# thu-nics/Rad-NeRF

Measured on AMD Instinct MI355X. Metric: million samples/s fwd+bwd, 8192 rays, model_zoo_size=2; rgb L∞ vs ref, higher is better.
Workload: dtype f16/f32

## Files before the change

include/radnerf.h:

```cpp
#ifndef RADNERF_H
#define RADNERF_H

#include <stdint.h>

#ifdef __cplusplus
extern "C" {
#endif

#define RN_ABI_VERSION 9
#define RN_FX_STATS_BYTES 640
int rn_version(void);
const char* rn_last_error(void);
const char* rn_abi_signatures(void);
void rn_set_debug_flags(int flags);
int rn_debug_cycles(unsigned long long* out);
int rn_set_level_pairing(uint64_t pairing);

int rn_ray_aabb_intersect(const float* rays_o, const float* rays_d, const float* centers,
                          const float* half_sizes, int64_t n_rays, int64_t n_voxels,
                          int32_t max_hits, int32_t* hit_cnt, float* hits_t,
                          int64_t* hits_voxel_idx, void* stream);

int rn_ray_sphere_intersect(const float* rays_o, const float* rays_d, const float* centers,
                            const float* radii, int64_t n_rays, int64_t n_spheres,
// ... 182 lines not shown
int rn_igrad_to_f32(int64_t n, int32_t* igrad_lo, int32_t* igrad_carry, const float* scale,
                    float* grid_grad, void* stream);

int rn_field_fwd_merged(const float* ts, const int32_t* ray_of, const float* rays_o,
                        const float* rays_d, const int32_t* seg_base, const int32_t* seg_count,
                        const int32_t* chunk_desc, int32_t* queue,
                        int64_t n_rays, int32_t n_models, const void* grid_f16,
                        const uint32_t* level_offset, const uint32_t* level_hsize,
                        const uint32_t* level_res, const float* level_scale,
                        const float* xyz_min, const float* extent, const void* frags,
                        float* sigma, float* rgb, void* feat_cache, const int32_t* mstart,
                        const int32_t* perm, int32_t blocks, int32_t threads, void* stream);

int rn_field_fwd_levels(const float* ts, const int32_t* ray_of, const float* rays_o,
                        const float* rays_d, const int32_t* seg_base, const int32_t* seg_count,
                        int64_t n_rays, int32_t n_models, const void* grid_f16,
                        const uint32_t* level_offset, const uint32_t* level_hsize,
                        const uint32_t* level_res, const float* level_scale,
                        const float* xyz_min, const float* extent, const void* frags,
                        float* sigma, float* rgb, void* feat_cache, const int32_t* mstart,
                        const int32_t* perm, uint32_t* planes, int64_t plane_stride, void* prep,
                        int32_t prep_ready, int32_t enc_blocks, int32_t mlp_blocks, int32_t* xq,
                        void* stream);

int rn_gate_fwd(const float* in0, const float* in1, int32_t stride, int64_t n_rays,
                int32_t n_models, const void* frags, float* gate, float* importance,
                int32_t n_blocks, void* stream);
int rn_gate_bwd(const float* in0, const float* in1, int32_t stride, int64_t n_rays,
                int32_t n_models, const void* frags, const float* dL_dgate, float* dw,
                int32_t n_params, const void* dinput_frags, float* dL_dinput,
                int32_t n_blocks, void* stream);

int rn_field_dinput(const float* xyzs, const float* dirs, int64_t n_samples, const float* ts,
                    const int32_t* ray_of, const float* rays_o, const float* rays_d,
                    const int32_t* seg_base, const int32_t* seg_count, int32_t n_models,
                    const void* grid_f16, const uint32_t* level_offset,
                    const uint32_t* level_hsize, const uint32_t* level_res,
                    const float* level_scale, const float* xyz_min, const float* extent,
                    const void* frags, const void* dinput_frags, const float* dL_dsigma,
                    const float* dL_drgb, const void* feat_cache, float* dL_dxyz,
                    float* dL_ddir, int32_t blocks_per_model, void* stream);
int rn_density_update_sampled(const void* grid_ptrs, const void* bitfield_ptrs, int32_t n_models,
                              int32_t cascades, int32_t grid_size, float scale,
                              float density_threshold, float decay, uint64_t seed,
                              const void* grid_f16, const uint32_t* level_offset,
                              const uint32_t* level_hsize, const uint32_t* level_res,
// ... 115 lines not shown
```

rad-nerf_amd/csrc/field.hip:

```cpp
#include "rn_field.h"
#include "rn_bin.h"
#include "rn_merge.h"
#include "rn_gradform.h"
#pragma clang fp contract(off)

static int g_field_dbg = 0;
__device__ unsigned long long g_rn_cyc[8];

namespace {

template <int MODE, int CACHE>
__global__ void __launch_bounds__(256, FWD_MIN_WAVES)
k_field_fwd(FieldArgs a) {
    __shared__ __attribute__((aligned(16))) rn_half sW[FIELD_FWD_FRAGS * RN_FRAG_HALFS];
    __shared__ LvTab sT;
    const int k = blockIdx.y;
    rn_block_copy16(sW, a.frags + (size_t)k * FIELD_FRAGS * RN_FRAG_HALFS,
                    FIELD_FWD_FRAGS * RN_FRAG_BYTES);
    lv_stage(sT, a.gm);
    __syncthreads();
    int64_t base, n;
    sample_range(a, MODE, k, base, n);
    const int64_t n_tiles = (n + 31) / 32;
    const int waves = blockDim.x / RN_WAVE;
// ... 1202 lines not shown
    return 0;
}

}
template <bool ABL, int DET>
static void launch_bwd_merged(int gm, int blocks, hipStream_t st, const FieldArgs& a,
                              const MergeArgs& m, const IntGrad& G, const FxGrad& F) {
#define MB_K(C, M) k_field_bwd_merged<C, ABL, M, DET><<<blocks, BWD_WAVES * 64, 0, st>>>(a, m, G, F)
    if constexpr (!DET) {
        if (gm == GM_BIN_F32) MB_K(CACHE_READ, GM_BIN_F32);
        if (gm == GM_BIN) MB_K(CACHE_READ, GM_BIN);
        if (gm == GM_FX) MB_K(CACHE_READ, GM_FX);
        if constexpr (!ABL) if (gm == GM_FX_REDO) MB_K(CACHE_READ, GM_FX_REDO);
    }
    if constexpr (!ABL) {
        if (gm == GM_INT) { if (a.feat) MB_K(CACHE_READ, GM_INT); else MB_K(CACHE_NONE, GM_INT); }
    }
    if constexpr (!DET) {
        if (gm == GM_F32) { if (a.feat) MB_K(CACHE_READ, GM_F32); else MB_K(CACHE_NONE, GM_F32); }
    }
#undef MB_K
}

static int field_bwd_merged(const char* who, bool det, const float* ts, const int32_t* ray_of,
                            const float* rays_o, const float* rays_d, const int32_t* seg_base,
                            const int32_t* seg_count, const int32_t* mstart, const int32_t* perm,
                            const int32_t* chunk_desc, int32_t* queue, int64_t n_rays,
                            int32_t n_models, int32_t max_samples, const void* grid_f16,
                            const uint32_t* level_offset, const uint32_t* level_hsize,
                            const uint32_t* level_res, const float* level_scale,
                            const float* xyz_min, const float* extent, const void* frags,
                            const float* dL_dsigma, const float* dL_drgb, float* grid_grad,
                            float* dw, const void* feat_cache, float* scratch,
                            int64_t scratch_rows, float* park, int32_t max_chunk, int32_t blocks,
                            int32_t* igrad_lo, int32_t* igrad_carry, const float* igrad_scale,
                            int32_t* fx_acc, const float* fx_scale, uint32_t* fx_stats,
                            const int32_t* fx_redo, int32_t fx_mode, void* gb_ctl,
                            uint32_t* gb_page_meta, uint64_t* gb_pages, int32_t gb_pool_pages,
                            void* stream) {
#define CHECK(cond, msg) RN_CHECK_ARG_AS(who, cond, msg)
    CHECK(!igrad_lo || (igrad_carry && igrad_scale), "integer mode needs carry and scale");
    CHECK(fx_mode >= GM_F32 && fx_mode <= GM_BIN_F32 && fx_mode != GM_INT, "fx_mode: 0, 2, 3, 4 or 5");
    const bool binned = gm_pages(fx_mode);
    CHECK(fx_mode != GM_FX || (fx_acc && fx_scale && fx_stats && feat_cache),
          "fixed-point mode needs acc, scale, stats and the encoding cache");
    CHECK(!binned || (fx_scale && fx_stats && feat_cache && gb_ctl && gb_page_meta && gb_pages &&
                      gb_pool_pages >= 1),
          "binned mode needs scale, stats, the encoding cache and the page pool");
    for (int l = 0; binned && l < RN_L; ++l)
        CHECK(level_hsize[l] <= (1u << GB_IDX_BITS) &&
              level_hsize[l] <= ((uint32_t)GB_MAX_BINS << GB_SLICE_BITS),
              "binned mode: a level has more than 2^20 entries");
    CHECK(fx_mode != GM_FX_REDO || (fx_redo && fx_scale && feat_cache),
          "fixed-point redo needs the redo flag, the step's scales and the encoding cache");
    CHECK(!(igrad_lo && fx_mode), "integer and fixed-point modes are exclusive");
    CHECK(n_rays >= 1 && n_models >= 1 && n_models <= MB_KMAX && blocks >= 1 &&
          max_samples >= 1 && max_chunk >= 1, "bad sizes");
    CHECK(scratch_rows >= (int64_t)max_chunk + (int64_t)n_models * max_samples,
          "scratch_rows must be >= max_chunk + n_models * max_samples");
    CHECK(ts && ray_of && rays_o && rays_d && seg_base && seg_count && mstart && perm &&
          chunk_desc && queue && grid_f16 && level_offset && level_hsize && level_res &&
          level_scale && xyz_min && extent && frags && dL_dsigma && dL_drgb && grid_grad && dw &&
          scratch && park, "null pointer");
    CHECK(fx_mode != GM_FX ||
          2ull * ((uint64_t)level_offset[RN_L - 1] + level_hsize[RN_L - 1]) <= (1ull << 28),
          "fixed-point mode: the grid has more than 2^28 gradient elements");
#undef CHECK
    FieldArgs a{};
    field_args_grid(a, grid_f16, level_offset, level_hsize, level_res, level_scale, xyz_min, extent,
                    frags);
    field_args_compact(a, ts, ray_of, rays_o, rays_d, seg_base, seg_count);
    a.dsigma = dL_dsigma; a.drgb = dL_drgb; a.grid_grad = grid_grad; a.dw = dw;
    a.feat = (rn_half*)feat_cache;
    MergeArgs m{};
    m.mstart = mstart; m.perm = perm; m.desc = chunk_desc; m.queue = queue; m.scratch = scratch;
    m.park = park; m.rows_cap = (int)scratch_rows; m.n_rays = (int)n_rays; m.n_models = n_models;
    hipStream_t st = (hipStream_t)stream;
    const size_t slots = (size_t)blocks * n_models * FIELD_PARAMS * sizeof(float);
    if (det) RN_CHECK_HIP_AS(who, hipMemsetAsync(dw, 0, slots, st), "dw_part reset");
    else RN_CHECK_HIP_AS(who, hipMemsetAsync(queue, 0, sizeof(int32_t), st), "ticket reset");
    IntGrad G{};
    if (igrad_lo) {
        G.bytes = 2 * a.grid_bytes;
        G.lo_ptr = igrad_lo; G.carry_ptr = igrad_carry; G.scale_ptr = igrad_scale;
    }
    if (binned) {
        RN_CHECK_HIP_AS(who, hipMemsetAsync(gb_ctl, 0, GB_CTL_RESET_BYTES, st), "page pool reset");
        G.ctl = (GbCtl*)gb_ctl; G.page_meta = gb_page_meta; G.pages = gb_pages;
        G.pool_pages = (uint32_t)gb_pool_pages;
    }
    FxGrad F{};
    F.acc = fx_acc; F.scale = fx_scale; F.redo = fx_redo;
    if (FxStats* S = reinterpret_cast<FxStats*>(fx_stats)) {
        F.vmax = S->vmax; F.qsum = S->qsum; F.wq = S->wq;
    }
    const int gm = fx_mode ? fx_mode : (igrad_lo ? GM_INT : GM_F32);
    const bool abl = RN_ABL && a.dbg && !det && gm != GM_INT && gm != GM_FX_REDO;
    if (abl) launch_bwd_merged<RN_ABL != 0, 0>(gm, blocks, st, a, m, G, F);
    else if (!det) launch_bwd_merged<false, 0>(gm, blocks, st, a, m, G, F);
    else launch_bwd_merged<false, 1>(gm, blocks, st, a, m, G, F);
    RN_CHECK_LAUNCH_AS(who);
    return 0;
}

extern "C" {
int rn_field_bwd_merged(const float* ts, const int32_t* ray_of, const float* rays_o,
                        const float* rays_d, const int32_t* seg_base, const int32_t* seg_count,
                        const int32_t* mstart, const int32_t* perm, const int32_t* chunk_desc,
                        int32_t* queue, int64_t n_rays, int32_t n_models, int32_t max_samples,
                        const void* grid_f16, const uint32_t* level_offset,
                        const uint32_t* level_hsize, const uint32_t* level_res,
                        const float* level_scale, const float* xyz_min, const float* extent,
                        const void* frags, const float* dL_dsigma, const float* dL_drgb,
                        float* grid_grad, float* dw, const void* feat_cache, float* scratch,
                        int64_t scratch_rows, float* park, int32_t max_chunk, int32_t blocks,
                        int32_t* igrad_lo, int32_t* igrad_carry, const float* igrad_scale,
                        int32_t* fx_acc, const float* fx_scale, uint32_t* fx_stats,
                        const int32_t* fx_redo, int32_t fx_mode, void* gb_ctl,
                        uint32_t* gb_page_meta, uint64_t* gb_pages, int32_t gb_pool_pages,
                        void* stream) {
    return field_bwd_merged(__func__, false, ts, ray_of, rays_o, rays_d, seg_base, seg_count,
// ... 10 lines not shown
                            const int32_t* seg_count, const int32_t* mstart, const int32_t* perm,
                            const int32_t* chunk_desc, const int32_t* queue, int64_t n_rays,
                            int32_t n_models, int32_t max_samples, const void* grid_f16,
                            const uint32_t* level_offset, const uint32_t* level_hsize,
                            const uint32_t* level_res, const float* level_scale,
                            const float* xyz_min, const float* extent, const void* frags,
                            const float* dL_dsigma, const float* dL_drgb, float* grid_grad,
                            float* dw_part, const void* feat_cache, float* scratch,
                            int64_t scratch_rows, float* park, int32_t max_chunk, int32_t blocks,
                            int32_t* igrad_lo, int32_t* igrad_carry, const float* igrad_scale,
                            void* stream) {
    RN_CHECK_ARG(igrad_lo && igrad_carry && igrad_scale,
                 "the deterministic backward needs igrad_lo, igrad_carry and igrad_scale");
    RN_CHECK_ARG(dw_part, "the deterministic backward needs dw_part");
    return field_bwd_merged(__func__, true, ts, ray_of, rays_o, rays_d, seg_base, seg_count,
                            mstart, perm, chunk_desc, const_cast<int32_t*>(queue), n_rays,
                            n_models, max_samples, grid_f16, level_offset, level_hsize, level_res,
                            level_scale, xyz_min, extent, frags, dL_dsigma, dL_drgb, grid_grad,
                            dw_part, feat_cache, scratch, scratch_rows, park, max_chunk, blocks,
                            igrad_lo, igrad_carry, igrad_scale, nullptr, nullptr, nullptr, nullptr,
                            GM_F32, nullptr, nullptr, nullptr, 0, stream);
}

}
```

rad-nerf_amd/csrc/field_fwd_merged.hip:

```cpp
#include "rn_field.h"
#include "rn_merge.h"
#pragma clang fp contract(off)

static uint64_t g_level_pairing = 0;

namespace {

#define FM_KMAX 8
#define FM_LDS_K 4
static_assert(FM_KMAX == MB_KMAX, "k_field_fwd_merged reads the plan's descriptors");

template <int CACHE, bool ENC_M, bool GW>
__global__ void __launch_bounds__(1024)
k_field_fwd_merged(FieldArgs a, MergeArgs m) {
    extern __shared__ __attribute__((aligned(16))) rn_half sWm[];
    __shared__ LvTab sT;
    __shared__ int32_t sCh[2][2 + 2 * FM_KMAX];
    const int K = m.n_models, B = m.n_rays;
    if (!GW) {
        for (int k = 0; k < K; ++k)
            rn_block_copy16(sWm + (size_t)k * FIELD_FWD_FRAGS * RN_FRAG_HALFS,
                            a.frags + (size_t)k * FIELD_FRAGS * RN_FRAG_HALFS,
                            FIELD_FWD_FRAGS * RN_FRAG_BYTES);
    }
// ... 182 lines not shown
            int k = kb;
            while (k < ke && u >= first[k + 1]) ++k;
            const int t = u - first[k];
            const int n_k = sSeg[1][k];
            const int i = t * 32 + c;
            const bool valid = i < n_k;
            const int64_t s = sSeg[0][k] + (valid ? i : 0);
            FwdState st;
            float ux, uy, uz;
            rn_lds_order();
            tile_forward_s<1, CACHE_PLANES>(a, sT, sWm + (size_t)(k - kb) * FIELD_FWD_FRAGS * RN_FRAG_HALFS,
                                            s, valid, a.feat ? cache_slot(a, s) : nullptr, st,
                                            ux, uy, uz);
            if (valid && h == 0) {
                a.sigma[s] = expf(st.g0);
                a.rgb[3 * s + 0] = sigmoidf(st.out[0]);
                a.rgb[3 * s + 1] = sigmoidf(st.out[1]);
                a.rgb[3 * s + 2] = sigmoidf(st.out[2]);
            }
        }
    }
}

}

extern "C" {

int rn_set_level_pairing(uint64_t pairing) {
    if (pairing != 0) {
        uint32_t seen = 0;
        for (int i = 0; i < 16; ++i) seen |= 1u << ((pairing >> (4 * i)) & 15u);
        RN_CHECK_ARG(seen == 0xffffu, "pairing: every level exactly once");
    }
    g_level_pairing = pairing;
    return 0;
}

int rn_field_fwd_merged(const float* ts, const int32_t* ray_of, const float* rays_o,
                        const float* rays_d, const int32_t* seg_base, const int32_t* seg_count,
                        const int32_t* chunk_desc, int32_t* queue,
                        int64_t n_rays, int32_t n_models, const void* grid_f16,
                        const uint32_t* level_offset, const uint32_t* level_hsize,
                        const uint32_t* level_res, const float* level_scale,
                        const float* xyz_min, const float* extent, const void* frags,
                        float* sigma, float* rgb, void* feat_cache, const int32_t* mstart,
                        const int32_t* perm, int32_t blocks, int32_t threads, void* stream) {
    RN_CHECK_ARG(n_rays >= 1 && n_models >= 1 && n_models <= FM_KMAX && blocks >= 1,
                 "bad sizes (n_models <= 8)");
    RN_CHECK_ARG(threads >= 64 && threads <= 1024 && threads % 64 == 0, "threads: 64..1024, waves");
// ... 76 lines not shown
```

rad-nerf_amd/csrc/rn_field.h:

```cpp
#pragma once
#include "rn_mlp.h"
#pragma clang fp contract(off)

#define RN_L 16
#define FIELD_FWD_FRAGS 24
#define FIELD_FRAGS 46
#define FIELD_PARAMS 9472
#define FIELD_DW_TILES 12
#ifndef FWD_MIN_WAVES
#define FWD_MIN_WAVES 2
#endif

struct GridMeta {
    uint32_t offset[RN_L];
    uint32_t hsize[RN_L];
    uint32_t res[RN_L];
    float scale[RN_L];
    uint32_t dense_mask;
    uint32_t pow2_mask;
};

struct FieldArgs {
    const float* xyzs; const float* dirs;
    const float* ts; const int32_t* ray_of; const float* rays_o; const float* rays_d;
// ... 401 lines not shown
template <int CACHE>
__device__ __forceinline__ void tile_forward_rays(const FieldArgs& a, const LvTab& T,
                                                  const rn_half* W, int64_t s, bool valid,
                                                  half8* fc, const float* sRays, int r0, int nr,
                                                  FwdState& st, float& ux, float& uy, float& uz) {
    float x = 0.f, y = 0.f, z = 0.f, dx = 1.f, dy = 0.f, dz = 0.f;
    if (valid) {
        const int r = a.ray_of[s];
        const float t = a.ts[s];
        const uint32_t q = (uint32_t)(r - r0);
        float ox, oy, oz;
        if (q < (uint32_t)nr) {
            typedef __attribute__((address_space(3))) const float lds_f;
            lds_f* p = (lds_f*)sRays + 6 * q;
            ox = p[0]; oy = p[1]; oz = p[2]; dx = p[3]; dy = p[4]; dz = p[5];
        } else {
            ox = a.rays_o[3 * r]; oy = a.rays_o[3 * r + 1]; oz = a.rays_o[3 * r + 2];
            dx = a.rays_d[3 * r]; dy = a.rays_d[3 * r + 1]; dz = a.rays_d[3 * r + 2];
        }
        x = fmaf(t, dx, ox);
        y = fmaf(t, dy, oy);
        z = fmaf(t, dz, oz);
    }
    tile_forward_pos<CACHE>(a, T, W, x, y, z, dx, dy, dz, valid, fc, st, ux, uy, uz);
}

template <int CACHE>
__device__ __forceinline__ void tile_forward_pos(const FieldArgs& a, const LvTab& T, const rn_half* W,
                                                 float x, float y, float z, float dx, float dy,
                                                 float dz, bool valid, half8* fc, FwdState& st,
                                                 float& ux, float& uy, float& uz) {
    const int h = rn_lane() >> 5;
    ux = unit_coord(x, a.xyz_min[0], a.extent[0]);
    uy = unit_coord(y, a.xyz_min[1], a.extent[1]);
    uz = unit_coord(z, a.xyz_min[2], a.extent[2]);
    if (CACHE == CACHE_PLANES) {
        if (valid && fc) { fc[0] = st.e0; fc[1] = st.e1; }
    } else if (CACHE == CACHE_READ || CACHE == CACHE_READ_NT) {
        st.e0 = rn_zero8(); st.e1 = rn_zero8();
        if (valid && CACHE == CACHE_READ) { st.e0 = fc[0]; st.e1 = fc[1]; }
        if (valid && CACHE == CACHE_READ_NT) {
            st.e0 = __builtin_nontemporal_load(fc);
            st.e1 = __builtin_nontemporal_load(fc + 1);
        }
    } else {
        if (rn_dbg(a.dbg) & 256) { st.e0 = rn_zero8(); st.e1 = rn_zero8(); asm volatile("" :: "v"(ux), "v"(uy), "v"(uz)); }
// ... 64 lines not shown
```

rad-nerf_amd/radnerf_amd/_lib.py:

```python
import ctypes
import os

_HERE = os.path.dirname(os.path.abspath(__file__))
LIB_PATH = os.environ.get("RADNERF_LIB", os.path.join(_HERE, "librn.so"))
ABLATION_LIB_PATH = os.environ.get("RADNERF_ABL_LIB", os.path.join(_HERE, "librn_abl.so"))

P = ctypes.c_void_p
I32 = ctypes.c_int32
I64 = ctypes.c_int64
F32 = ctypes.c_float
F64 = ctypes.c_double
U64 = ctypes.c_uint64

SIGNATURES = {
    "rn_ray_aabb_intersect": [P, P, P, P, I64, I64, I32, P, P, P, P],
    "rn_ray_sphere_intersect": [P, P, P, P, I64, I64, I32, P, P, P, P],
    "rn_raymarching_train_bw": [P, P, P, P, I64, P, P, P],
    "rn_ml_march_bw": [P, P, I64, I32, P, P, P, P, P, P],
    "rn_field_dinput": [P, P, I64, P, P, P, P, P, P, I32, P, P, P, P, P, P, P, P, P, P, P, P, P,
                        P, I32, P],
    "rn_field_density": [P, I64, P, P, P, P, P, P, P, P, P, P, P],
    "rn_debug_cycles": [P],
    "rn_set_level_pairing": [ctypes.c_uint64],
    "rn_density_update_sampled": [P, P, I32, I32, I32, F32, F32, F32, U64, P, P, P, P, P, P, P,
# ... 28 lines not shown
    "rn_bwd_plan": [P, P, P, P, P, I64, I32, I32, I32, I32, I32, I32, I32, P, P, P, P, P,
                    P, P, P, P, P, P],
    "rn_field_bwd_merged": [P, P, P, P, P, P, P, P, P, P, I64, I32, I32, P, P, P, P, P, P,
                            P, P, P, P, P, P, P, P, I64, P, I32, I32, P, P, P, P, P, P,
                            P, I32, P, P, P, I32, P],
    "rn_grid_fx_fold": [P, P, P, P, P, P, P, P, P, P],
    "rn_grid_bin_layout": [P],
    "rn_debug_gb_cycles": [P],
    "rn_grid_slice_bits": [P, P],
    "rn_grid_record_encode": [P, I64, P],
    "rn_grid_record_decode": [P, I64, P],
    "rn_grid_bin": [P, P, P, P, P, P, P, I32, I32, P],
    "rn_grid_sum": [P, P, P, P, P, P, I32, P, P, P, I32, I32, P],
    "rn_grid_bin_check": [P, P, P, P, P, P, P, I32, P, P, P, P, P],
    "rn_grid_binned_fold": [P, P, P, P, P, P, P, P, I32, P, P, P, P, P, P],
    "rn_render_test": [P, P, P, I64, I32, P, I64, I32, F32, F32, I32, I32, P, P, P, P, P, P, P,
                       P, F32, P, P, P, P, I32, P],
    "rn_seed_scale": [P, P, I32, P, P, P, P, P, P],
    "rn_igrad_to_f32": [I64, P, P, P, P, P],
    "rn_field_fwd_merged": [P, P, P, P, P, P, P, P, I64, I32, P, P, P, P, P, P, P, P, P, P, P,
                            P, P, I32, I32, P],
    "rn_field_fwd_levels": [P, P, P, P, P, P, I64, I32, P, P, P, P, P, P, P, P, P, P, P, P, P,
                            P, I64, P, I32, I32, I32, P, P],
    "rn_gate_fwd": [P, P, I32, I64, I32, P, P, P, I32, P],
    "rn_gate_bwd": [P, P, I32, I64, I32, P, P, P, I32, P, P, I32, P],
    "rn_nerf_loss": [P, P, P, P, P, P, I64, I32, F32, F32, F32, P, P, P, P, P, P],
    "rn_adam": [P, P, P, P, I64, F64, F64, F64, F64, I32, F32, P, I64, P],
    "rn_reduce_partials": [P, I32, I64, P, P],
    "rn_colsum_ordered": [P, I64, I32, P, P],
    "rn_field_bwd_merged_det": [P, P, P, P, P, P, P, P, P, P, I64, I32, I32, P, P, P, P, P, P,
                                P, P, P, P, P, P, P, P, I64, P, I32, I32, P, P, P, P],
    "rn_gate_bwd_det": [P, P, I32, I64, I32, P, P, P, I32, P, P, I32, P],
    "rn_nerf_loss_det": [P, P, P, P, P, P, I64, I32, F32, F32, F32, P, P, P, P, P, P, P],
    "rn_get_rays": [P, P, P, P, I64, P, P, P, P, P],
    "rn_get_rays_pose": [P, P, P, P, P, P, I64, P, P, P, P, P],
    "rn_get_rays_pose_bw": [P, P, P, P, P, I64, I64, P, P, P, P, P, P, P],
    "rn_sample_batch": [P, I32, I64, I64, P, P, P, P, P, U64, I64, I32, I64, I32, P, P, P, P, P,
                        P, P, P, P],
    "rn_ml_combine_test": [P, P, P, P, P, I64, I32, I64, P, P, P, P, P],
    "rn_image_sse": [P, P, I64, P, P, P],
    "rn_ssim": [P, P, I32, I32, I32, P, P, P, P],
    "rn_minmax_finite": [P, I64, I64, P, P, P],
    "rn_quantize_u8": [P, I64, P, P],
    "rn_colormap_u8": [P, I64, I64, P, P, I32, P, P],
    "rn_gate_map_u8": [P, I64, I32, P, I32, P, P],
    "rn_pack_f16": [P, I64, P, I64, I32, I64, P, P],
# ... 115 lines not shown
```

rad-nerf_amd/radnerf_amd/fused.py:

```python
import collections

import torch

from . import layout as LY
from ._lib import lib
from .networks import field_ptrs, model_bitfields

MAX_SAMPLES = 1024
NEAR_DISTANCE = 0.01
SEG_ALIGN = 128
FX_STATS_BYTES = 640
GM_F32, GM_FX, GM_FX_REDO, GM_BIN, GM_BIN_F32 = 0, 2, 3, 4, 5
NO_IG, NO_FX, NO_GB = (None, None, None), (None, None, None, None, GM_F32), (None, None, None, 0)


GB_SUM_FAULT = 18
GB_CTL_READ = GB_SUM_FAULT + 1


def clamp_split(split_level):
    return max(0, min(15, int(split_level)))


def _stream(dev):
# ... 10 lines not shown
        self.B, self.K, self.device = B, K, device
        cap = capacity or (B * K * max_samples + SEG_ALIGN * K)
        self.capacity = cap
        f = dict(device=device, dtype=torch.float32)
        i = dict(device=device, dtype=torch.int32)
        self.counts = torch.empty(K, B, **i)
        self.offsets = torch.empty(K, B, **i)
        self.seg = torch.zeros(2 * K + 2, **i)
        self.used = torch.empty(K, B, **i)
        self.ts = torch.empty(cap, **f)
        self.deltas = torch.empty(cap, **f)
        self.ray_of = torch.empty(cap, **i)
        self.sigma = torch.empty(cap, **f)
        self.rgb = torch.empty(cap, 3, **f)
        self.ws = torch.empty(cap, **f)
        self.dsigma = torch.empty(cap, **f)
        self.drgb = torch.empty(cap, 3, **f)
        self.opacity_k = torch.empty(K, B, **f)
        self.depth_k = torch.empty(K, B, **f)
        self.rgb_k = torch.empty(K, B, 3, **f)
        self.dgate = torch.empty(B, K, **f)
        self.stage_ts = torch.empty(K * B * max_samples, **f)
        self.stage_dt = torch.empty(K * B * max_samples, **f)
        self.feat = torch.empty((cap + 31) // 32 * 32, 32, device=device, dtype=torch.float16)
        self.mstart = torch.empty(B + 1, **i)
        self.perm = torch.empty(cap, **i)
        self.queue = torch.zeros(3, **i)
        self._bwd_scratch = None
        self._chunks = self._chunk_desc = None
        self._dist_k = None
        self._igrad = self._fx = self._bin = self._bin_ring = None
        self.fx_i = self._bin_n = 0
        self.dw_part = self.gate_part = None
        self.gate_dx = self.dxyz = self.ddir = self.drays_o = self.drays_d = None
        self.generation = 0

    @property
    def dist_k(self):
        if self._dist_k is None:
            self._dist_k = torch.empty(self.K, self.B, device=self.device, dtype=torch.float32)
        return self._dist_k

    def chunk_list(self, max_chunk, min_chunk, head_chunks=0, balance_blocks=0):
        cap = (head_chunks + self.capacity // max_chunk + self.capacity // (8 * min_chunk) +
               max_chunk // min_chunk + 3 + balance_blocks)
        if self._chunks is None or self._chunks.numel() < cap + 1:
            self._chunks = torch.empty(cap + 1, device=self.device, dtype=torch.int32)
            self._chunk_desc = torch.empty(cap + 1, 20, device=self.device, dtype=torch.int32)
        return cap, self._chunks

    def level_buffers(self, stream=None):
        rows = self.feat.shape[0]
        key = (str(self.device), int(stream) if stream is not None else 0)
        cur = _LEVEL_SCRATCH.get(key)
        if cur is None or cur[0].shape[1] < rows:
            cur = (torch.empty(16, rows, device=self.device, dtype=torch.int32),
                   torch.empty(rows, 4, device=self.device, dtype=torch.float32))
            _LEVEL_SCRATCH[key] = cur
        return cur

    def fx_buffers(self, n, device):
        if self._fx is None or self._fx[0].numel() != n:
            z = dict(device=device, dtype=torch.int32)
            self._fx = (torch.zeros(n, **z), torch.zeros(2, 16, device=device),
                        torch.zeros(FX_STATS_BYTES // 4, **z), torch.zeros(1, **z))
            self.fx_i = 0
        return self._fx

    def bin_pool(self, pages):
        b = self._bin
        if b is None or b["pages"] < pages:
            lay = lib().bin_layout()
            i = dict(device=self.device, dtype=torch.int32)
            self._bin = b = dict(
                pages=pages, page=lay["page"],
                ctl=torch.zeros(lay["ctl_bytes"] // 4, **i),
                meta=torch.zeros(pages, **i),
                recs=torch.empty(pages * lay["page"], device=self.device, dtype=torch.int64),
                desc=torch.empty(pages * lay["bins"], **i),
                lpages=torch.empty(16 * pages, **i))
        return b

# ... 17 lines not shown
    @property
    def meta(self):
        return self.seg[2 * self.K:]

    def n_samples(self):
        return int(self.meta[1].item())


class FusedMLRenderer:

    def __init__(self, model, gating_net, n_rays, device=None, fwd_blocks=None, bwd_blocks=None,
                 capacity=None, deterministic=False):
        self._deterministic = self._merged_bwd = False
        if deterministic and not 1 <= model.size <= 8:
            raise ValueError(self._NO_DET + f" (this model: {model.size} sub-NeRFs)")
        self.model, self.gate = model, gating_net
        self.device = device or model.mlp_params.device
        self.ws = Workspace(n_rays, model.size, self.device, capacity=capacity)
        K = model.size
        self.bitfield_bytes = model_bitfields(model)[0].numel()
        self.fwd_blocks = fwd_blocks or max(1, 2048 // K)
        self.bwd_blocks = bwd_blocks or max(1, 256 // K)
        self.feat_cache = True
        self.merged_bwd = 1 <= model.size <= 8
        self.merged_fwd = 1 < model.size <= 8
        self.merged_encode = model.size > 1
        self.merged_fwd_blocks = 256
        self.merged_fwd_threads = 1024
        self.level_fwd = self.merged_bwd or self.merged_fwd
        self.plan_prep = True
        self.level_enc_blocks = 4096
        self.level_mlp_blocks = 256
        self.merged_blocks = 256
        rk = n_rays * model.size
        self.max_chunk = 256 if rk <= 1024 else (512 if rk <= 4096 else 1024)
        if model.size >= 8 and rk > 4096:
            self.max_chunk = 12288
        elif model.size >= 4 and rk > 4096 and float(model.scale) > 0.5:
            self.max_chunk = 4096
        elif model.size >= 2 and rk > 4096 and float(model.scale) <= 0.5:
            self.max_chunk = 1536
        self.int_grad = False
        self.deterministic = bool(deterministic)
        self.grid_fx = rk > 1024
        self.grid_bin = self.grid_fx and float(model.scale) > 0.5
        self.bin_f32_levels = (9 if model.size >= 8 else 8) if self.grid_bin else 0
# ... 33 lines not shown
            raise ValueError(self._NO_DET)
        self._merged_bwd = bool(on)

    @property
    def deterministic(self):
        return self._deterministic

    @deterministic.setter
    def deterministic(self, on):
        if on and not self._merged_bwd:
            raise ValueError(self._NO_DET + f" (this renderer: {self.model.size} sub-NeRFs, "
                             f"merged_bwd {self._merged_bwd})")
        self._deterministic = bool(on)

    @property
    def scatter_mode(self):
        if not self.merged_bwd:
            return "fp32-atomics"
        if self.int_grad or self.deterministic:
            return "int-grad"
        if self.grid_fx and self.feat_cache:
            return "binned" if self.grid_bin else "fixed-point"
        return "fp32-atomics"

    def _ev(self, name, L_call, *args, stream=None):
        if not self.trace or (self.trace is not True and name not in self.trace):
            return L_call(*args)
        a, b = torch.cuda.Event(enable_timing=True), torch.cuda.Event(enable_timing=True)
        a.record(stream)
        L_call(*args)
        b.record(stream)
        self.events.setdefault(name, []).append((a, b))

    def _ev_open(self, name):
        if not self.trace or (self.trace is not True and name not in self.trace):
            return None
        a = torch.cuda.Event(enable_timing=True)
        a.record()
        return (name, a)

    def _ev_close(self, span):
        if span is not None:
            b = torch.cuda.Event(enable_timing=True)
            b.record()
            self.events.setdefault(span[0], []).append((span[1], b))

# ... 107 lines not shown
                 w.seg_base.data_ptr(), w.seg_count.data_ptr(), w.ts.data_ptr(), w.B, w.K,
                 head_n, head, max_chunk, min_chunk, bal, self._cap_chunks,
                 w.mstart.data_ptr(), w.perm.data_ptr(), self._chunks.data_ptr(),
                 w._chunk_desc.data_ptr(), w.queue.data_ptr(),
                 *((None,) * 5 if prep is None else
                   (rays_o.data_ptr(), rays_d.data_ptr(), m._h_min.ctypes.data,
                    m._h_ext.ctypes.data, prep.data_ptr())), st)
        self._plan_key = key
        self._prep_ready = prep is not None

    def _sample_ptrs(self, rays_o, rays_d):
        w = self.ws
        return (w.ts.data_ptr(), w.ray_of.data_ptr(), rays_o.data_ptr(), rays_d.data_ptr(),
                w.seg_base.data_ptr(), w.seg_count.data_ptr())

    def _field(self, fwd, rays_o, rays_d, st, grid_grad=None, dw=None):
        return (self._field_fwd(rays_o, rays_d, st) if fwd else
                self._field_bwd(rays_o, rays_d, st, grid_grad, dw))

    def _field_fwd(self, rays_o, rays_d, st):
        m, w, L = self.model, self.ws, lib()
        samples, grid = self._sample_ptrs(rays_o, rays_d), field_ptrs(m)
        out = (w.sigma.data_ptr(), w.rgb.data_ptr())
        feat = w.feat.data_ptr() if self.feat_cache else None
        if self.level_fwd and (self.merged_bwd or self.merged_fwd):
            planes, prep = w.level_buffers(st)
            self._ev("field_fwd", L.field_fwd_levels, *samples, w.B, m.size, *grid, *out,
                     w.feat.data_ptr(), w.mstart.data_ptr(), w.perm.data_ptr(),
                     planes.data_ptr(), planes.shape[1], prep.data_ptr(), int(self._prep_ready),
                     self.level_enc_blocks, self.level_mlp_blocks, None, st)
            self._prep_ready = False
        elif self.merged_fwd:
            order = ((w.mstart.data_ptr(), w.perm.data_ptr())
                     if self.feat_cache and self.merged_encode else (None, None))
            self._ev("field_fwd", L.field_fwd_merged, *samples, w._chunk_desc.data_ptr(),
                     w.queue.data_ptr(), w.B, m.size, *grid, *out, feat, *order,
                     self.merged_fwd_blocks, self.merged_fwd_threads, st)
        else:
            self._ev("field_fwd", L.field_fwd, None, None, 0, *samples, m.size, *grid, *out, feat,
                     self.fwd_blocks, st)

    def _field_bwd(self, rays_o, rays_d, st, grid_grad, dw):
        m, w, L = self.model, self.ws, lib()
        samples, grid = self._sample_ptrs(rays_o, rays_d), field_ptrs(m)
        feat = w.feat.data_ptr() if self.feat_cache else None
        if not self.merged_bwd:
            return self._bwd_f32(lambda name: self._ev(
                name, L.field_bwd, None, None, 0, *samples, m.size, *grid, w.dsigma.data_ptr(),
                w.drgb.data_ptr(), grid_grad.data_ptr(), dw.data_ptr(), feat, self.bwd_blocks, st))
        rows, scratch, park = w.bwd_scratch(self.merged_blocks, self.max_chunk)
        if self._plan_key != self._plan_params():
            self._plan(st)
        head = (*samples, w.mstart.data_ptr(), w.perm.data_ptr(), w._chunk_desc.data_ptr(),
                w.queue.data_ptr(), w.B, m.size, MAX_SAMPLES, *grid, w.dsigma.data_ptr(),
                w.drgb.data_ptr(), grid_grad.data_ptr())
        tail = (feat, scratch.data_ptr(), rows, park.data_ptr(), self.max_chunk, self.merged_blocks)

        def launch(name, ig=NO_IG, fx=NO_FX, gb=NO_GB, dw_part=None):
            if dw_part is not None:
                self._ev(name, L.field_bwd_merged_det, *head, dw_part.data_ptr(), *tail, *ig, st)
            else:
                self._ev(name, L.field_bwd_merged, *head, dw.data_ptr(), *tail, *ig, *fx, *gb, st)

        form = {"int-grad": self._bwd_int, "fixed-point": self._bwd_fx,
                "binned": self._bwd_binned, "fp32-atomics": self._bwd_f32}[self.scatter_mode]
        form(launch, grid_grad, dw, st)

    @staticmethod
    def _hook(fn, *args):
        if fn is not None:
            fn(*args)

    def _bwd_f32(self, launch, *_):
        launch("field_bwd")
        self._hook(self.after_field_bwd)
        self._hook(self.after_grid_levels, 0)

    def _igrad_buffers(self, grid_grad):
        w, n_g = self.ws, grid_grad.numel()
        if w._igrad is None or w._igrad[0].numel() != n_g:
            z = dict(device=grid_grad.device, dtype=torch.int32)
            w._igrad = (torch.zeros(n_g, **z), torch.zeros(n_g, **z),
                        torch.ones(1, device=grid_grad.device), torch.zeros(1, **z))
# ... 214 lines not shown
        if w.dxyz is None:
            w.dxyz = torch.empty(w.capacity, 3, device=w.device)
            w.ddir = torch.empty(w.capacity, 3, device=w.device)
            w.drays_o = torch.empty(w.B, 3, device=w.device)
            w.drays_d = torch.empty(w.B, 3, device=w.device)
        self._ev("field_dinput", L.field_dinput, None, None, 0,
                 *self._sample_ptrs(rays_o, rays_d), m.size, *field_ptrs(m),
                 m.packed_dinput_frags().data_ptr(), w.dsigma.data_ptr(), w.drgb.data_ptr(),
                 w.feat.data_ptr() if self.feat_cache else None, w.dxyz.data_ptr(),
                 w.ddir.data_ptr(), self.fwd_blocks, st)
        self._ev("march_bw", L.ml_march_bw, w.counts.data_ptr(), w.offsets.data_ptr(), w.B, m.size,
                 w.ts.data_ptr(), w.dxyz.data_ptr(), w.ddir.data_ptr(), w.drays_o.data_ptr(),
                 w.drays_d.data_ptr(), st)

    def _dgate(self, B, G):
        return self.ws.dgate

    def train_step(self, rays_o, rays_d, gate_in2, target_rgb, noise, bg, lambda_opacity=1e-3,
                   lambda_cv_importance=0.0, lambda_depth_mutual=0.0, T_threshold=1e-4,
                   exp_step_factor=0.0, grid_grad=None, mlp_grad=None, gate_grad=None,
                   lambda_distortion=0.0, input_grad=False):
        from .losses import fused_nerf_loss
        dist = lambda_distortion > 0
        rgb, opacity, depth, gate, imp = self.forward(rays_o, rays_d, gate_in2, noise, bg,
                                                      T_threshold, exp_step_factor, dist)
        self.last_forward = {"rgb": rgb, "opacity": opacity, "depth": depth, "gate": gate,
                             "importance": imp}
        terms, (d_rgb, d_op, d_depth, d_gate) = fused_nerf_loss(
            rgb, target_rgb, opacity, depth, gate, imp, lambda_opacity, lambda_cv_importance,
            lambda_depth_mutual, lambda_distortion, self.ws.dist_k if dist else None,
            deterministic=self.deterministic)
        d_dist = float(lambda_distortion) / rays_o.shape[0] if dist else None
        if not input_grad:
            grads = self.backward(rays_o, rays_d, gate_in2, gate, bg, d_rgb, d_op, d_depth,
                                  d_gate, T_threshold, grid_grad, mlp_grad, gate_grad, d_dist)
            return terms, grads
        saved, self.input_grad = self.input_grad, True
        try:
            grads = self.backward(rays_o, rays_d, gate_in2, gate, bg, d_rgb, d_op, d_depth,
                                  d_gate, T_threshold, grid_grad, mlp_grad, gate_grad, d_dist)
        finally:
            self.input_grad = saved
        w = self.ws
        return terms, grads, (w.drays_o + w.gate_dx[:, 0:3], w.drays_d, w.gate_dx[:, 3:6])


class _MLRenderFn(torch.autograd.Function):
    @staticmethod
    def forward(ctx, grid_params, mlp_params, gate_params, renderer, rays_o, rays_d, gate_in2,
                noise, bg, T_threshold, esf, distortion=False):
        rgb, opacity, depth, gate, imp = renderer.forward(rays_o, rays_d, gate_in2, noise, bg,
                                                          T_threshold, esf, distortion)
        renderer.ws.generation += 1
        ctx.generation = renderer.ws.generation
        ctx.renderer = renderer
        ctx.save_for_backward(rays_o, rays_d, gate_in2, gate, bg)
        ctx.T = T_threshold
        if distortion:
            return rgb, opacity, depth, gate, renderer.ws.dist_k.t().contiguous()
        return rgb, opacity, depth, gate

    @staticmethod
    def backward(ctx, d_rgb, d_op, d_depth, d_gate, d_dist=None):
        rays_o, rays_d, gate_in2, gate, bg = ctx.saved_tensors
        if ctx.renderer.ws.generation != ctx.generation:
            raise RuntimeError(
                "ml_render_fused: the renderer's workspace was reused by another forward "
                "(same model, gate and batch size) before this backward; run the backward "
                "first, or render the other batch under torch.no_grad()")
        B, K = gate.shape
        dev = rays_o.device
        z = lambda *s: torch.zeros(*s, device=dev)
        d_rgb = z(B, 3) if d_rgb is None else d_rgb.float().contiguous()
        d_op = z(B) if d_op is None else d_op.float().contiguous()
        d_depth = None if d_depth is None else d_depth.float().contiguous()
# ... 100 lines not shown
```

Measured before the change: 1201.

## Read level planes directly in merged backward instead of writing a feature cache

The level-wise forward already writes encodings into per-level planes. This change lets the merged backward read those planes with buffer loads and drops the separate interleaved feature-cache write during forward when only fixed-point or binned scatter is used. The cache is rebuilt lazily by a new conversion kernel only if another consumer asks for it. This removes a large forward write and a buffer, in exchange for strided per-level loads in backward and extra state tracking for staleness.

```diff
diff --git a/include/radnerf.h b/include/radnerf.h
--- a/include/radnerf.h
+++ b/include/radnerf.h
@@ -228,6 +228,26 @@
                         const int32_t* perm, uint32_t* planes, int64_t plane_stride, void* prep,
                         int32_t prep_ready, int32_t enc_blocks, int32_t mlp_blocks, int32_t* xq,
                         void* stream);
+
+int rn_field_bwd_merged_planes(const float* ts, const int32_t* ray_of, const float* rays_o,
+                               const float* rays_d, const int32_t* seg_base,
+                               const int32_t* seg_count, const int32_t* mstart,
+                               const int32_t* perm, const int32_t* chunk_desc, int32_t* queue,
+                               int64_t n_rays, int32_t n_models, int32_t max_samples,
+                               const void* grid_f16, const uint32_t* level_offset,
+                               const uint32_t* level_hsize, const uint32_t* level_res,
+                               const float* level_scale, const float* xyz_min,
+                               const float* extent, const void* frags, const float* dL_dsigma,
+                               const float* dL_drgb, float* grid_grad, float* dw,
+                               const void* feat_cache, float* scratch, int64_t scratch_rows,
+                               float* park, int32_t max_chunk, int32_t blocks, int32_t* igrad_lo,
+                               int32_t* igrad_carry, const float* igrad_scale, int32_t* fx_acc,
+                               const float* fx_scale, uint32_t* fx_stats, const int32_t* fx_redo,
+                               int32_t fx_mode, void* gb_ctl, uint32_t* gb_page_meta,
+                               uint64_t* gb_pages, int32_t gb_pool_pages, void* stream,
+                               const uint32_t* planes, int64_t plane_stride);
+int rn_planes_to_cache(const uint32_t* planes, int64_t plane_stride, int64_t n_slots,
+                       void* feat_cache, void* stream);
 
 int rn_gate_fwd(const float* in0, const float* in1, int32_t stride, int64_t n_rays,
                 int32_t n_models, const void* frags, float* gate, float* importance,
diff --git a/rad-nerf_amd/csrc/field.hip b/rad-nerf_amd/csrc/field.hip
--- a/rad-nerf_amd/csrc/field.hip
+++ b/rad-nerf_amd/csrc/field.hip
@@ -1248,6 +1248,9 @@
 #undef MB_K
 }
 
+static void launch_bwd_merged_planes(int gm, int blocks, hipStream_t st, const FieldArgs& a,
+                                     const MergeArgs& m, const IntGrad& G, const FxGrad& F);
+
 static int field_bwd_merged(const char* who, bool det, const float* ts, const int32_t* ray_of,
                             const float* rays_o, const float* rays_d, const int32_t* seg_base,
                             const int32_t* seg_count, const int32_t* mstart, const int32_t* perm,
@@ -1263,21 +1266,23 @@
                             int32_t* fx_acc, const float* fx_scale, uint32_t* fx_stats,
                             const int32_t* fx_redo, int32_t fx_mode, void* gb_ctl,
                             uint32_t* gb_page_meta, uint64_t* gb_pages, int32_t gb_pool_pages,
-                            void* stream) {
+                            void* stream, const uint32_t* planes = nullptr,
+                            int64_t plane_stride = 0) {
 #define CHECK(cond, msg) RN_CHECK_ARG_AS(who, cond, msg)
+    const bool enc = feat_cache || planes;
     CHECK(!igrad_lo || (igrad_carry && igrad_scale), "integer mode needs carry and scale");
     CHECK(fx_mode >= GM_F32 && fx_mode <= GM_BIN_F32 && fx_mode != GM_INT, "fx_mode: 0, 2, 3, 4 or 5");
     const bool binned = gm_pages(fx_mode);
-    CHECK(fx_mode != GM_FX || (fx_acc && fx_scale && fx_stats && feat_cache),
+    CHECK(fx_mode != GM_FX || (fx_acc && fx_scale && fx_stats && enc),
           "fixed-point mode needs acc, scale, stats and the encoding cache");
-    CHECK(!binned || (fx_scale && fx_stats && feat_cache && gb_ctl && gb_page_meta && gb_pages &&
+    CHECK(!binned || (fx_scale && fx_stats && enc && gb_ctl && gb_page_meta && gb_pages &&
                       gb_pool_pages >= 1),
           "binned mode needs scale, stats, the encoding cache and the page pool");
     for (int l = 0; binned && l < RN_L; ++l)
         CHECK(level_hsize[l] <= (1u << GB_IDX_BITS) &&
               level_hsize[l] <= ((uint32_t)GB_MAX_BINS << GB_SLICE_BITS),
               "binned mode: a level has more than 2^20 entries");
-    CHECK(fx_mode != GM_FX_REDO || (fx_redo && fx_scale && feat_cache),
+    CHECK(fx_mode != GM_FX_REDO || (fx_redo && fx_scale && enc),
           "fixed-point redo needs the redo flag, the step's scales and the encoding cache");
     CHECK(!(igrad_lo && fx_mode), "integer and fixed-point modes are exclusive");
     CHECK(n_rays >= 1 && n_models >= 1 && n_models <= MB_KMAX && blocks >= 1 &&
@@ -1298,6 +1303,7 @@
     field_args_compact(a, ts, ray_of, rays_o, rays_d, seg_base, seg_count);
     a.dsigma = dL_dsigma; a.drgb = dL_drgb; a.grid_grad = grid_grad; a.dw = dw;
     a.feat = (rn_half*)feat_cache;
+    a.planes = planes; a.plane_stride = plane_stride;
     MergeArgs m{};
     m.mstart = mstart; m.perm = perm; m.desc = chunk_desc; m.queue = queue; m.scratch = scratch;
     m.park = park; m.rows_cap = (int)scratch_rows; m.n_rays = (int)n_rays; m.n_models = n_models;
@@ -1322,7 +1328,9 @@
     }
     const int gm = fx_mode ? fx_mode : (igrad_lo ? GM_INT : GM_F32);
     const bool abl = RN_ABL && a.dbg && !det && gm != GM_INT && gm != GM_FX_REDO;
-    if (abl) launch_bwd_merged<RN_ABL != 0, 0>(gm, blocks, st, a, m, G, F);
+    if (planes && !det && gm != GM_INT && gm != GM_F32)
+        launch_bwd_merged_planes(gm, blocks, st, a, m, G, F);
+    else if (abl) launch_bwd_merged<RN_ABL != 0, 0>(gm, blocks, st, a, m, G, F);
     else if (!det) launch_bwd_merged<false, 0>(gm, blocks, st, a, m, G, F);
     else launch_bwd_merged<false, 1>(gm, blocks, st, a, m, G, F);
     RN_CHECK_LAUNCH_AS(who);
@@ -1379,4 +1387,47 @@
                             GM_F32, nullptr, nullptr, nullptr, 0, stream);
 }
 
-}
+int rn_field_bwd_merged_planes(const float* ts, const int32_t* ray_of, const float* rays_o,
+                               const float* rays_d, const int32_t* seg_base,
+                               const int32_t* seg_count, const int32_t* mstart,
+                               const int32_t* perm, const int32_t* chunk_desc, int32_t* queue,
+                               int64_t n_rays, int32_t n_models, int32_t max_samples,
+                               const void* grid_f16, const uint32_t* level_offset,
+                               const uint32_t* level_hsize, const uint32_t* level_res,
+                               const float* level_scale, const float* xyz_min,
+                               const float* extent, const void* frags, const float* dL_dsigma,
+                               const float* dL_drgb, float* grid_grad, float* dw,
+                               const void* feat_cache, float* scratch, int64_t scratch_rows,
+                               float* park, int32_t max_chunk, int32_t blocks, int32_t* igrad_lo,
+                               int32_t* igrad_carry, const float* igrad_scale, int32_t* fx_acc,
+                               const float* fx_scale, uint32_t* fx_stats, const int32_t* fx_redo,
+                               int32_t fx_mode, void* gb_ctl, uint32_t* gb_page_meta,
+                               uint64_t* gb_pages, int32_t gb_pool_pages, void* stream,
+                               const uint32_t* planes, int64_t plane_stride) {
+    RN_CHECK_ARG(planes || feat_cache, "needs the level planes or the encoding cache");
+    if (planes) {
+        RN_CHECK_ARG(plane_stride >= 1, "plane_stride must be >= 1");
+        RN_CHECK_ARG((uint64_t)plane_stride * (RN_L * 4u) < (1ull << 32),
+                     "the level planes (16 x plane_stride x 4 B) must be below 4 GB");
+    }
+    return field_bwd_merged(__func__, false, ts, ray_of, rays_o, rays_d, seg_base, seg_count,
+                            mstart, perm, chunk_desc, queue, n_rays, n_models, max_samples,
+                            grid_f16, level_offset, level_hsize, level_res, level_scale, xyz_min,
+                            extent, frags, dL_dsigma, dL_drgb, grid_grad, dw, feat_cache, scratch,
+                            scratch_rows, park, max_chunk, blocks, igrad_lo, igrad_carry,
+                            igrad_scale, fx_acc, fx_scale, fx_stats, fx_redo, fx_mode, gb_ctl,
+                            gb_page_meta, gb_pages, gb_pool_pages, stream, planes,
+                            planes ? plane_stride : 0);
+}
+
+}
+
+static void launch_bwd_merged_planes(int gm, int blocks, hipStream_t st, const FieldArgs& a,
+                                     const MergeArgs& m, const IntGrad& G, const FxGrad& F) {
+#define MB_P(M) k_field_bwd_merged<CACHE_PLANES, false, M, 0><<<blocks, BWD_WAVES * 64, 0, st>>>(a, m, G, F)
+    if (gm == GM_BIN_F32) MB_P(GM_BIN_F32);
+    if (gm == GM_BIN) MB_P(GM_BIN);
+    if (gm == GM_FX) MB_P(GM_FX);
+    if (gm == GM_FX_REDO) MB_P(GM_FX_REDO);
+#undef MB_P
+}
diff --git a/rad-nerf_amd/csrc/field_fwd_merged.hip b/rad-nerf_amd/csrc/field_fwd_merged.hip
--- a/rad-nerf_amd/csrc/field_fwd_merged.hip
+++ b/rad-nerf_amd/csrc/field_fwd_merged.hip
@@ -228,9 +228,37 @@
     }
 }
 
+__global__ void __launch_bounds__(256)
+k_planes_to_cache(const uint32_t* __restrict__ planes, int64_t stride, int64_t n_slots,
+                  uint4* __restrict__ feat) {
+    const int64_t i = (int64_t)blockIdx.x * blockDim.x + threadIdx.x;
+    const int lane = (int)(i & 63), c = lane & 31, h = lane >> 5;
+    const int64_t s = (i >> 6) * 32 + c;
+    if (s >= n_slots) return;
+    uint32_t w[8];
+#pragma unroll
+    for (int q = 0; q < 8; ++q) w[q] = planes[(int64_t)lane_level(q, h) * stride + s];
+    feat[2 * i] = make_uint4(w[0], w[1], w[2], w[3]);
+    feat[2 * i + 1] = make_uint4(w[4], w[5], w[6], w[7]);
+}
+
 }
 
 extern "C" {
+
+int rn_planes_to_cache(const uint32_t* planes, int64_t plane_stride, int64_t n_slots,
+                       void* feat_cache, void* stream) {
+    RN_CHECK_ARG(planes && feat_cache, "null pointer");
+    RN_CHECK_ARG(plane_stride >= 1 && n_slots >= 0 && n_slots <= plane_stride,
+                 "bad sizes (0 <= n_slots <= plane_stride)");
+    if (n_slots == 0) return 0;
+    const int64_t threads = (n_slots + 31) / 32 * 64;
+    RN_CHECK_ARG((threads + 255) / 256 < (1ll << 31), "too many slots for one launch");
+    k_planes_to_cache<<<(unsigned)((threads + 255) / 256), 256, 0, (hipStream_t)stream>>>(
+        planes, plane_stride, n_slots, (uint4*)feat_cache);
+    RN_CHECK_LAUNCH();
+    return 0;
+}
 
 int rn_set_level_pairing(uint64_t pairing) {
     if (pairing != 0) {
diff --git a/rad-nerf_amd/csrc/rn_field.h b/rad-nerf_amd/csrc/rn_field.h
--- a/rad-nerf_amd/csrc/rn_field.h
+++ b/rad-nerf_amd/csrc/rn_field.h
@@ -447,6 +447,20 @@
         y = fmaf(t, dy, oy);
         z = fmaf(t, dz, oz);
     }
+    if (CACHE == CACHE_PLANES) {
+        const int h = rn_lane() >> 5;
+        const uint32_t sb = (uint32_t)a.plane_stride * 4u;
+        const __amdgpu_buffer_rsrc_t prs = rn_rsrc(a.planes, 16u * sb);
+        const uint32_t vo = valid ? ((uint32_t)s << 2) + (h ? 2u * sb : 0u) : 0xfffffffcu;
+        typedef uint32_t u4v __attribute__((ext_vector_type(4)));
+        u4v w0, w1;
+#pragma unroll
+        for (int q = 0; q < 4; ++q) {
+            w0[q] = __builtin_amdgcn_raw_buffer_load_b32(prs, vo, ((q & 1) + 4 * (q >> 1)) * sb, 0);
+            w1[q] = __builtin_amdgcn_raw_buffer_load_b32(prs, vo, (8 + (q & 1) + 4 * (q >> 1)) * sb, 0);
+        }
+        st.e0 = __builtin_bit_cast(half8, w0); st.e1 = __builtin_bit_cast(half8, w1);
+    }
     tile_forward_pos<CACHE>(a, T, W, x, y, z, dx, dy, dz, valid, fc, st, ux, uy, uz);
 }
 
diff --git a/rad-nerf_amd/radnerf_amd/_lib.py b/rad-nerf_amd/radnerf_amd/_lib.py
--- a/rad-nerf_amd/radnerf_amd/_lib.py
+++ b/rad-nerf_amd/radnerf_amd/_lib.py
@@ -74,6 +74,10 @@
                             P, P, I32, I32, P],
     "rn_field_fwd_levels": [P, P, P, P, P, P, I64, I32, P, P, P, P, P, P, P, P, P, P, P, P, P,
                             P, I64, P, I32, I32, I32, P, P],
+    "rn_field_bwd_merged_planes": [P, P, P, P, P, P, P, P, P, P, I64, I32, I32, P, P, P, P, P, P,
+                                   P, P, P, P, P, P, P, P, I64, P, I32, I32, P, P, P, P, P, P,
+                                   P, I32, P, P, P, I32, P, P, I64],
+    "rn_planes_to_cache": [P, I64, I64, P, P],
     "rn_gate_fwd": [P, P, I32, I64, I32, P, P, P, I32, P],
     "rn_gate_bwd": [P, P, I32, I64, I32, P, P, P, I32, P, P, I32, P],
     "rn_nerf_loss": [P, P, P, P, P, P, I64, I32, F32, F32, F32, P, P, P, P, P, P],
diff --git a/rad-nerf_amd/radnerf_amd/fused.py b/rad-nerf_amd/radnerf_amd/fused.py
--- a/rad-nerf_amd/radnerf_amd/fused.py
+++ b/rad-nerf_amd/radnerf_amd/fused.py
@@ -56,7 +56,10 @@
         self.dgate = torch.empty(B, K, **f)
         self.stage_ts = torch.empty(K * B * max_samples, **f)
         self.stage_dt = torch.empty(K * B * max_samples, **f)
-        self.feat = torch.empty((cap + 31) // 32 * 32, 32, device=device, dtype=torch.float16)
+        self.rows = (cap + 31) // 32 * 32
+        self._feat = self._planes = None
+        self.feat_stale = False
+        self.planes_fresh = False
         self.mstart = torch.empty(B + 1, **i)
         self.perm = torch.empty(cap, **i)
         self.queue = torch.zeros(3, **i)
@@ -83,15 +86,29 @@
             self._chunk_desc = torch.empty(cap + 1, 20, device=self.device, dtype=torch.int32)
         return cap, self._chunks
 
+    def feat_buffer(self):
+        if self._feat is None:
+            self._feat = torch.empty(self.rows, 32, device=self.device, dtype=torch.float16)
+        return self._feat
+
+    @property
+    def feat(self):
+        feat = self.feat_buffer()
+        if self.feat_stale and self._planes is not None:
+            lib().planes_to_cache(self._planes.data_ptr(), self.rows, self.rows, feat.data_ptr(),
+                                  _stream(self.device))
+        self.feat_stale = False
+        return feat
+
     def level_buffers(self, stream=None):
-        rows = self.feat.shape[0]
+        if self._planes is None:
+            self._planes = torch.empty(16, self.rows, device=self.device, dtype=torch.int32)
         key = (str(self.device), int(stream) if stream is not None else 0)
-        cur = _LEVEL_SCRATCH.get(key)
-        if cur is None or cur[0].shape[1] < rows:
-            cur = (torch.empty(16, rows, device=self.device, dtype=torch.int32),
-                   torch.empty(rows, 4, device=self.device, dtype=torch.float32))
-            _LEVEL_SCRATCH[key] = cur
-        return cur
+        prep = _LEVEL_SCRATCH.get(key)
+        if prep is None or prep.shape[0] < self.rows:
+            prep = torch.empty(self.rows, 4, device=self.device, dtype=torch.float32)
+            _LEVEL_SCRATCH[key] = prep
+        return self._planes, prep
 
     def fx_buffers(self, n, device):
         if self._fx is None or self._fx[0].numel() != n:
@@ -155,6 +172,7 @@
         self.fwd_blocks = fwd_blocks or max(1, 2048 // K)
         self.bwd_blocks = bwd_blocks or max(1, 256 // K)
         self.feat_cache = True
+        self.plane_bwd = True
         self.merged_bwd = 1 <= model.size <= 8
         self.merged_fwd = 1 < model.size <= 8
         self.merged_encode = model.size > 1
@@ -234,6 +252,13 @@
         if self.grid_fx and self.feat_cache:
             return "binned" if self.grid_bin else "fixed-point"
         return "fp32-atomics"
+
+    def _planes_bwd_ok(self):
+        return bool(self.plane_bwd and self.scatter_mode in ("fixed-point", "binned") and
+                    self.ws.rows * 64 < (1 << 32))
+
+    def planes_only(self):
+        return bool(self._planes_bwd_ok() and self.level_fwd and not self.input_grad)
 
     def _ev(self, name, L_call, *args, stream=None):
         if not self.trace or (self.trace is not True and name not in self.trace):
@@ -387,15 +412,19 @@
         m, w, L = self.model, self.ws, lib()
         samples, grid = self._sample_ptrs(rays_o, rays_d), field_ptrs(m)
         out = (w.sigma.data_ptr(), w.rgb.data_ptr())
-        feat = w.feat.data_ptr() if self.feat_cache else None
         if self.level_fwd and (self.merged_bwd or self.merged_fwd):
             planes, prep = w.level_buffers(st)
+            only = self.planes_only()
             self._ev("field_fwd", L.field_fwd_levels, *samples, w.B, m.size, *grid, *out,
-                     w.feat.data_ptr(), w.mstart.data_ptr(), w.perm.data_ptr(),
-                     planes.data_ptr(), planes.shape[1], prep.data_ptr(), int(self._prep_ready),
-                     self.level_enc_blocks, self.level_mlp_blocks, None, st)
+                     None if only else w.feat_buffer().data_ptr(), w.mstart.data_ptr(),
+                     w.perm.data_ptr(), planes.data_ptr(), planes.shape[1], prep.data_ptr(),
+                     int(self._prep_ready), self.level_enc_blocks, self.level_mlp_blocks, None, st)
             self._prep_ready = False
-        elif self.merged_fwd:
+            w.feat_stale, w.planes_fresh = only, True
+            return
+        feat = w.feat_buffer().data_ptr() if self.feat_cache else None
+        w.feat_stale = w.planes_fresh = False
+        if self.merged_fwd:
             order = ((w.mstart.data_ptr(), w.perm.data_ptr())
                      if self.feat_cache and self.merged_encode else (None, None))
             self._ev("field_fwd", L.field_fwd_merged, *samples, w._chunk_desc.data_ptr(),
@@ -408,7 +437,8 @@
     def _field_bwd(self, rays_o, rays_d, st, grid_grad, dw):
         m, w, L = self.model, self.ws, lib()
         samples, grid = self._sample_ptrs(rays_o, rays_d), field_ptrs(m)
-        feat = w.feat.data_ptr() if self.feat_cache else None
+        planes = w._planes if w.planes_fresh and self._planes_bwd_ok() else None
+        feat = None if planes is not None or not self.feat_cache else w.feat.data_ptr()
         if not self.merged_bwd:
             return self._bwd_f32(lambda name: self._ev(
                 name, L.field_bwd, None, None, 0, *samples, m.size, *grid, w.dsigma.data_ptr(),
@@ -424,6 +454,9 @@
         def launch(name, ig=NO_IG, fx=NO_FX, gb=NO_GB, dw_part=None):
             if dw_part is not None:
                 self._ev(name, L.field_bwd_merged_det, *head, dw_part.data_ptr(), *tail, *ig, st)
+            elif planes is not None:
+                self._ev(name, L.field_bwd_merged_planes, *head, dw.data_ptr(), *tail, *ig, *fx,
+                         *gb, st, planes.data_ptr(), planes.shape[1])
             else:
                 self._ev(name, L.field_bwd_merged, *head, dw.data_ptr(), *tail, *ig, *fx, *gb, st)
 
@@ -684,8 +717,12 @@
                    lambda_distortion=0.0, input_grad=False):
         from .losses import fused_nerf_loss
         dist = lambda_distortion > 0
-        rgb, opacity, depth, gate, imp = self.forward(rays_o, rays_d, gate_in2, noise, bg,
-                                                      T_threshold, exp_step_factor, dist)
+        saved, self.input_grad = self.input_grad, self.input_grad or bool(input_grad)
+        try:
+            rgb, opacity, depth, gate, imp = self.forward(rays_o, rays_d, gate_in2, noise, bg,
+                                                          T_threshold, exp_step_factor, dist)
+        finally:
+            self.input_grad = saved
         self.last_forward = {"rgb": rgb, "opacity": opacity, "depth": depth, "gate": gate,
                              "importance": imp}
         terms, (d_rgb, d_op, d_depth, d_gate) = fused_nerf_loss(
@@ -711,8 +748,13 @@
     @staticmethod
     def forward(ctx, grid_params, mlp_params, gate_params, renderer, rays_o, rays_d, gate_in2,
                 noise, bg, T_threshold, esf, distortion=False):
-        rgb, opacity, depth, gate, imp = renderer.forward(rays_o, rays_d, gate_in2, noise, bg,
-                                                          T_threshold, esf, distortion)
+        saved = renderer.input_grad
+        renderer.input_grad = saved or any(ctx.needs_input_grad[4:7])
+        try:
+            rgb, opacity, depth, gate, imp = renderer.forward(rays_o, rays_d, gate_in2, noise, bg,
+                                                              T_threshold, esf, distortion)
+        finally:
+            renderer.input_grad = saved
         renderer.ws.generation += 1
         ctx.generation = renderer.ws.generation
         ctx.renderer = renderer
```

New measurement: 1208 (median of 6 runs). No clear change (+0.6%).
